# tensorflow/compression

Measured on NVIDIA H100. Metric: range-code throughput (bls2017 compress path, cfg2), higher is better.
Workload: dtype u32

## Files before the change

compression_b200/csrc/range_coder.cu:

```cuda
#include <algorithm>
#include <cstring>
#include <vector>

#include <cstring>
#include <mutex>
#include <vector>

#include "common.cuh"

namespace tfcb {
namespace {

constexpr unsigned kFull = 0xFFFFFFFFu;

struct HostRow {
  int32_t start;
  int32_t ncdf;
  int32_t prec;
};

__host__ __device__ inline int row_ncdf(int meta) { return meta & 0xFFFFFF; }
__host__ __device__ inline int row_prec(int meta) { return (meta >> 24) & 0x1F; }
__host__ __device__ inline bool row_ovf(int meta) { return meta < 0; }

// ... 78 lines not shown
    if (for_decoder) {
      hr4.resize(meta.size());
      for (size_t i = 0; i < hr.size(); ++i) {
        const int ap = hr[i].prec < 0 ? -hr[i].prec : hr[i].prec;
        const int n = hr[i].ncdf - 1;
        const int pstart = (int)hp.size();
        int median = n, irregular = 0;
        for (int e = 0; e <= n; ++e) {
          const uint32_t c = (uint32_t)lookup_host[hr[i].start + e];
          hp.push_back((c == (1u << ap)) ? make_uint2(0xFFFFFFFFu, 0u) : make_uint2(c << (32 - ap), 0xFFFFFFFFu));
          if (e >= 1 && c == 0u) irregular = 1;
          if (e >= 1 && e < n && c == (1u << ap)) irregular = 1;
          if (e >= 1 && median == n && c >= (1u << ap) / 2) median = e;
        }
        for (int e = n + 1; e <= 64; ++e) hp.push_back(make_uint2(0xFFFFFFFFu, 0u));
        int wfirst = median - 31;
        if (wfirst > n - 63) wfirst = n - 63;
        if (wfirst < 1) wfirst = 1;
        hr4[i] = make_int4(pstart, meta[i].y, wfirst, irregular);
      }
      zero_win = (int)hp.size();
      for (int e = 0; e < 64; ++e) hp.push_back(make_uint2(0u, 0u));
      n_pairs = (long long)hp.size();
      TFCB_TRY(dev_alloc((void**)&pairs, hp.size() * sizeof(uint2), s));
      TFCB_TRY(dev_alloc((void**)&rows4, hr4.size() * sizeof(int4), s));
      TFCB_CUDA_TRY(cudaMemcpyAsync(pairs, hp.data(), hp.size() * sizeof(uint2), cudaMemcpyHostToDevice, s));
      TFCB_CUDA_TRY(cudaMemcpyAsync(rows4, hr4.data(), hr4.size() * sizeof(int4), cudaMemcpyHostToDevice, s));
    }
    TFCB_CUDA_TRY(cudaStreamSynchronize(s));
    return TFCB_OK;
  }
  void release(cudaStream_t s) {
    dev_free(lookup, s);
    dev_free(rows, s);
    dev_free(pairs, s);
    dev_free(rows4, s);
    lookup = nullptr;
    rows = nullptr;
    pairs = nullptr;
    rows4 = nullptr;
  }
};

struct EncState {
  uint32_t base;
  uint32_t span;
  uint32_t cnt;
  uint32_t raw;
};

__host__ __device__ inline EncState enc_initial_state() {
  EncState s;
  s.base = 0;
  s.span = 0xFFFFFFFFu;
  s.cnt = 0;
  s.raw = 0xFFFFFFFFu;
  return s;
}


__device__ __forceinline__ uint4 enc_operands(uint32_t lower, uint32_t upper, uint32_t p) {
  const uint32_t sh = 16u - p;
  return make_uint4(lower << sh, 0u, upper << sh, 0u);
}

struct EncChain {
  uint32_t s;

  __device__ __forceinline__ uint2 step(uint2 ol, uint2 oh) {
    const unsigned long long ql = (unsigned long long)s * ol.x + (((unsigned long long)ol.y << 32) | ol.x);
    const unsigned long long qu = (unsigned long long)s * oh.x + (((unsigned long long)oh.y << 32) | oh.x);
    const uint32_t shift = (s < 65536u) ? 0u : 16u;
    const uint32_t L = __funnelshift_r((uint32_t)ql, (uint32_t)(ql >> 32), shift);
    const uint32_t U = __funnelshift_r((uint32_t)qu, (uint32_t)(qu >> 32), shift);
    asm("{\n\t.reg .u32 t;\n\tsub.u32 t, %1, %2;\n\tsub.u32 %0, t, 1;\n\t}" : "=r"(s) : "r"(U), "r"(L));
    return make_uint2(L, s);
  }
  __device__ __forceinline__ uint2 step(uint4 o) { return step(make_uint2(o.x, o.y), make_uint2(o.z, o.w)); }
};

__device__ __forceinline__ uint32_t shl_clamp(uint32_t x, uint32_t s) { return __funnelshift_lc(0u, x, s); }

struct EncDrain {
  uint32_t dbase;
  uint32_t cnt;
  uint32_t cb_cur;
  uint16_t* words;
  uint32_t* cbits;
  uint32_t cap;
  bool overflowed;
  int lane;

  __device__ __forceinline__ void begin(const EncState& st, uint16_t* w, uint32_t* cb, uint32_t cap_, int lane_) {
    dbase = st.base;
    cnt = st.cnt;
    words = w;
    cbits = cb;
    cap = cap_;
    overflowed = false;
    lane = lane_;
    cb_cur = (st.cnt == 0) ? 0u : cb[st.cnt >> 5];
  }

  template <int kPasses>
  __device__ __forceinline__ void drain(const uint2* ent, int n) {
    uint32_t Lk[kPasses], Ak[kPasses], Sk[kPasses], rmask[kPasses];
#pragma unroll
    for (int p = 0; p < kPasses; ++p) {
      const int k = p * 32 + lane;
      const bool act = k < n;
      const uint2 me = ent[act ? k : 0];
      const bool rr = act && me.y < 65536u;
      rmask[p] = __ballot_sync(kFull, rr);
      Lk[p] = act ? me.x : 0u;
      uint32_t S = rr ? 16u : 0u;
      uint32_t A = Lk[p] << S;
#pragma unroll
      for (int d = 1; d < 32; d <<= 1) {
        const uint32_t Ap = __shfl_up_sync(kFull, A, d);
        const uint32_t Sp = __shfl_up_sync(kFull, S, d);
        if (lane >= d) {
          A = shl_clamp(Ap, S) + A;
          S = min(Sp + S, 32u);
        }
      }
      Ak[p] = A;
      Sk[p] = S;
    }
#pragma unroll
    for (int p = 0; p < kPasses; ++p) {
      if (p * 32 >= n) break;
      uint32_t Ax = __shfl_up_sync(kFull, Ak[p], 1);
      uint32_t Sx = __shfl_up_sync(kFull, Sk[p], 1);
      if (lane == 0) {
        Ax = 0u;
        Sx = 0u;
      }
      const uint32_t before = shl_clamp(dbase, Sx) + Ax;
      const uint32_t nb = before + Lk[p];
      const bool carry = nb < before;
      const bool ren = (rmask[p] >> lane) & 1u;
      const uint32_t my_cnt = cnt + __popc(rmask[p] & ((1u << lane) - 1u));
      if (ren) {
        if (my_cnt < cap) words[my_cnt] = (uint16_t)(nb >> 16);
        else overflowed = true;
      }
      const uint32_t g0 = cnt >> 5;
      const uint32_t bit = 1u << (my_cnt & 31u);
      const uint32_t m0 = __reduce_or_sync(kFull, (carry && (my_cnt >> 5) == g0) ? bit : 0u);
      const uint32_t m1 = __reduce_or_sync(kFull, (carry && (my_cnt >> 5) != g0) ? bit : 0u);
      const uint32_t pass_end = cnt + __popc(rmask[p]);
      cb_cur |= m0;
      if ((pass_end >> 5) != g0) {
        if (lane == 0 && g0 < (cap >> 5)) cbits[g0] = cb_cur;
        cb_cur = m1;
      }
      cnt = pass_end;
      dbase = shl_clamp(dbase, __shfl_sync(kFull, Sk[p], 31)) + __shfl_sync(kFull, Ak[p], 31);
    }
  }

  __device__ __forceinline__ void end(DevError* err, long long stream) {
    if ((cnt >> 5) < (cap >> 5)) {
      if (lane == 0) cbits[cnt >> 5] = cb_cur;
    } else {
      overflowed = true;
    }
    if (__any_sync(kFull, overflowed)) report(err, kErrCapacity, stream, cnt, cnt, cap);
  }
};

enum : int { kModeIndex = 1, kModeF32 = 2, kModeDecoded = 4 };

struct EncParams {
  const int32_t* lookup;
  const int2* rows;
  int n_rows;
  int uniform_prec;
  const void* value;
  const int32_t* index;
  const float* qoff;
  const int32_t* coff;
  long long n;
  long long n_streams;
  int fresh;
  EncState* state;
  uint16_t* words;
  uint32_t* cbits;
  long long cap;
  DevError* err;
  const long long* sym_off;
  const long long* arena_off;
  float* decoded;
};

struct Extent {
  long long base, len;
};
__device__ __forceinline__ Extent stream_extent(const long long* off, long long s, long long stride) {
  if (off) return Extent{off[s], off[s + 1] - off[s]};
  return Extent{s * stride, stride};
}

struct Fetched {
  float y;
  int v;
  float loc_or_q;
  int coff;
  int row;
  int2 ri;
  bool valid;
};

struct Gathered {
  uint4 ops;
  uint32_t prec;
  uint32_t gamma;
  uint32_t sign;
};

template <int MODE>
__device__ __forceinline__ Fetched enc_fetch(const EncParams& P, long long end, long long at, uint32_t chan_row) {
  Fetched f;
  f.y = 0.f;
  f.v = 0;
  f.loc_or_q = 0.f;
  f.coff = 0;
  f.row = (int)chan_row;
  f.ri = make_int2(0, 0);
  f.valid = at < end;
  if (!f.valid) return f;
  if (MODE & kModeF32) {
    f.y = __ldg(reinterpret_cast<const float*>(P.value) + at);
  } else {
    f.v = __ldg(reinterpret_cast<const int32_t*>(P.value) + at);
  }
  if (MODE & kModeIndex) {
    f.row = __ldg(P.index + at);
    if ((MODE & kModeF32) && P.qoff) f.loc_or_q = __ldg(P.qoff + at);
  } else {
    f.ri = __ldg(P.rows + f.row);
    if (MODE & kModeF32) {
      if (P.qoff) f.loc_or_q = __ldg(P.qoff + f.row);
      f.coff = __ldg(P.coff + f.row);
    }
  }
  return f;
}

template <int MODE>
__device__ __forceinline__ Gathered enc_gather(const EncParams& P, long long s, long long at, Fetched f) {
  Gathered g;
  g.ops = make_uint4(0u, 0u, 0u, 0u);
  g.prec = 0;
  g.gamma = 0;
  g.sign = 0;
  if (!f.valid) return g;
  if (MODE & kModeIndex) {
    if (f.row < 0 || f.row >= P.n_rows) {
      report(P.err, kErrIndex, s, at - stream_extent(P.sym_off, s, P.n).base, f.row, P.n_rows);
      return g;
    }
    f.ri = __ldg(P.rows + f.row);
    if (MODE & kModeF32) f.coff = __ldg(P.coff + f.row);
  }
  int v = f.v;
  if (MODE & kModeF32) v = (int)rintf(f.y - f.loc_or_q) - f.coff;
  if (MODE & kModeDecoded) {
    float yv = (float)(v + f.coff);
    if (P.qoff) yv += f.loc_or_q;
    P.decoded[at] = yv;
  }
  const int ncdf = row_ncdf(f.ri.y);
  if (!row_ovf(f.ri.y)) {
    if (v < 0 || v >= ncdf - 1) {
      report(P.err, kErrValue, s, at - stream_extent(P.sym_off, s, P.n).base, v, ncdf - 1);
      return g;
    }
  } else {
    const int esc = ncdf - 2;
    if (v < 0) {
      g.gamma = (uint32_t)(-(long long)v);
      g.sign = 1;
      v = esc;
    } else if (v >= esc) {
      g.gamma = (uint32_t)(v - esc + 1);
      v = esc;
    }
  }
  const uint32_t lower = (uint32_t)__ldg(P.lookup + f.ri.x + v);
  const uint32_t upper = (uint32_t)__ldg(P.lookup + f.ri.x + v + 1);
  g.prec = (uint32_t)row_prec(f.ri.y);
  g.ops = enc_operands(lower, upper, g.prec);
  return g;
}

__device__ __forceinline__ void bar_sync(int id, int count) {
  asm volatile("bar.sync %0, %1;" ::"r"(id), "r"(count) : "memory");
}
__device__ __forceinline__ void bar_arrive(int id, int count) {
  asm volatile("bar.arrive %0, %1;" ::"r"(id), "r"(count) : "memory");
}

constexpr int kBlock = 256;

struct BlockInfo {
  uint32_t n;
  uint32_t last;
};

constexpr int kPrefetch = 4;
static_assert(kPrefetch == 2 || kPrefetch == 4 || kPrefetch == 8, "the chain loop unrolls by 8 records");

struct EncShared {
  uint4 ops[2][kBlock + kPrefetch];
  uint2 ent[2][kBlock];
  BlockInfo ops_info[2];
  BlockInfo ent_info[2];
};

enum : int { kBarOpsFull = 1, kBarOpsEmpty = 3, kBarEntFull = 5, kBarEntEmpty = 7 };

struct RecordWriter {
  EncShared* sh;
  long long blocks;
  int fill;

  __device__ __forceinline__ void begin(EncShared* sh_) {
    sh = sh_;
    blocks = 0;
    fill = 0;
  }
  __device__ __forceinline__ uint4* cur() { return sh->ops[blocks & 1]; }
  __device__ __forceinline__ void publish(bool last) {
    const int b = (int)(blocks & 1);
    if ((threadIdx.x & 31) == 0) {
      BlockInfo bi;
      bi.n = (uint32_t)fill;
      bi.last = last ? 1u : 0u;
      sh->ops_info[b] = bi;
    }
    bar_arrive(kBarOpsFull + b, 64);
    ++blocks;
    fill = 0;
    if (!last && blocks >= 2) bar_sync(kBarOpsEmpty + (int)(blocks & 1), 64);
  }
  template <typename F>
  __device__ __forceinline__ void append(uint4 first, int pre, int extra, int total, bool has, F rec) {
    int done = 0;
    while (done < total) {
      const int room = kBlock - fill;
      const int take = min(room, total - done);
      uint4* dst = cur() + fill - done;
      if (has) {
        if (pre >= done && pre < done + take) dst[pre] = first;
        for (int i = 0; i < extra; ++i) {
          const int at = pre + 1 + i;
          if (at >= done && at < done + take) dst[at] = rec(i);
        }
      }
      fill += take;
      done += take;
      if (fill == kBlock) publish(false);
    }
  }
};

__device__ __forceinline__ uint4 gamma_record(uint32_t g, uint32_t sign, int nb, int i) {
  uint32_t bit;
  if (i < nb - 1) bit = 0u;
  else if (i < 2 * nb - 1) bit = (g >> (2 * nb - 2 - i)) & 1u;
  else bit = sign;
  return enc_operands(bit, bit + 1u, 1u);
}

template <int MODE>
__global__ void __launch_bounds__(192) encode_kernel(const EncParams P) {
  __shared__ __align__(16) EncShared sh;
  const long long s = blockIdx.x;
  const int lane = threadIdx.x & 31;
  const int warp = threadIdx.x >> 5;
  if (warp != 0 && warp != 1 && warp != 5) return;

  if (warp == 1) {
    uint32_t row_a = 0, chan_step = 0;
    if (!(MODE & kModeIndex)) {
      row_a = (uint32_t)lane % (uint32_t)P.n_rows;
      chan_step = 32u % (uint32_t)P.n_rows;
    }
    auto advance_row = [&]() {
      if (!(MODE & kModeIndex)) {
        row_a += chan_step;
        if (row_a >= (uint32_t)P.n_rows) row_a -= (uint32_t)P.n_rows;
      }
    };
    const Extent x = stream_extent(P.sym_off, s, P.n);
    const long long end = x.base + x.len;
    Fetched f0 = enc_fetch<MODE>(P, end, x.base + lane, row_a);
    advance_row();
    Fetched f1 = enc_fetch<MODE>(P, end, x.base + 32 + lane, row_a);
    advance_row();
    Fetched f2 = enc_fetch<MODE>(P, end, x.base + 64 + lane, row_a);
    advance_row();
    RecordWriter w;
    w.begin(&sh);
    bool stop = false;
    for (long long j0 = x.base; j0 < end && !stop; j0 += 32) {
      const Fetched fcur = f0;
      f0 = f1;
      f1 = f2;
      f2 = enc_fetch<MODE>(P, end, j0 + 96 + lane, row_a);
      advance_row();
      const Gathered cur = enc_gather<MODE>(P, s, j0 + lane, fcur);
      const int count = (int)min(32ll, end - j0);
      const bool has = lane < count;
      const unsigned esc_mask = __ballot_sync(kFull, cur.gamma != 0);
      const unsigned bad_mask = __ballot_sync(kFull, cur.prec == 0 && has);
      if (bad_mask) {
        stop = true;
        break;
      }
      if (esc_mask == 0) {
        if (w.fill + count <= kBlock) {
          if (has) w.cur()[w.fill + lane] = cur.ops;
          w.fill += count;
          if (w.fill == kBlock) w.publish(false);
        } else {
          w.append(cur.ops, lane, 0, count, has, [&](int) { return cur.ops; });
        }
      } else {
        const int nb = cur.gamma ? 32 - __clz(cur.gamma) : 0;
        const int mine = has ? 1 + 2 * nb : 0;
        int incl = mine;
#pragma unroll
        for (int d = 1; d < 32; d <<= 1) {
          const int t = __shfl_up_sync(kFull, incl, d);
          if (lane >= d) incl += t;
        }
        const int total = __shfl_sync(kFull, incl, 31);
        w.append(cur.ops, incl - mine, 2 * nb, total, has,
                 [&](int i) { return gamma_record(cur.gamma, cur.sign, nb, i); });
      }
    }
    w.publish(true);
    return;
  }

  if (warp == 5) {
    EncDrain d;
    const Extent a = stream_extent(P.arena_off, s, P.cap);
    d.begin(P.fresh ? enc_initial_state() : P.state[s], P.words + a.base, P.cbits + (a.base >> 5), (uint32_t)a.len,
            lane);
    for (long long k = 0;; ++k) {
      const int b = (int)(k & 1);
      bar_sync(kBarEntFull + b, 64);
      const BlockInfo bi = sh.ent_info[b];
      d.drain<kBlock / 32>(sh.ent[b], (int)bi.n);
      if (bi.last) break;
      bar_arrive(kBarEntEmpty + b, 64);
    }
    d.end(P.err, s);
    if (lane == 0) {
      P.state[s].base = d.dbase;
      P.state[s].cnt = d.cnt;
    }
    return;
  }

  EncChain c;
  c.s = P.fresh ? enc_initial_state().raw : P.state[s].raw;
  for (long long k = 0;; ++k) {
    const int b = (int)(k & 1);
    bar_sync(kBarOpsFull + b, 64);
    const BlockInfo bi = sh.ops_info[b];
    if (k >= 2) bar_sync(kBarEntEmpty + b, 64);
    const uint2* q = reinterpret_cast<const uint2*>(sh.ops[b]);
    uint2* e = sh.ent[b];
    const int n = (int)bi.n;
    int kk = 0;
    uint2 lo[kPrefetch], hi[kPrefetch];
#pragma unroll
    for (int r = 0; r < kPrefetch; ++r) {
      lo[r] = q[2 * r];
      hi[r] = q[2 * r + 1];
    }
#pragma unroll 1
    for (; kk + 8 <= n; kk += 8) {
      const uint2* p = q + 2 * kk;
      uint2* const eo = e + kk;
#pragma unroll
      for (int j = 0; j < 8; j += 2) {
        const int r0 = j % kPrefetch, r1 = (j + 1) % kPrefetch;
        const uint2 a0 = lo[r0], b0 = hi[r0], a1 = lo[r1], b1 = hi[r1];
        lo[r0] = p[2 * (j + kPrefetch)];
        hi[r0] = p[2 * (j + kPrefetch) + 1];
        lo[r1] = p[2 * (j + 1 + kPrefetch)];
        hi[r1] = p[2 * (j + 1 + kPrefetch) + 1];
        eo[j] = c.step(a0, b0);
        eo[j + 1] = c.step(a1, b1);
      }
    }
    for (; kk < n; ++kk) e[kk] = c.step(sh.ops[b][kk]);
    if (lane == 0) sh.ent_info[b] = bi;
    bar_arrive(kBarEntFull + b, 64);
    if (bi.last) break;
    bar_arrive(kBarOpsEmpty + b, 64);
  }
  if (lane == 0) {
    P.state[s].span = (c.s < 65536u) ? ((c.s << 16) | 0xFFFFu) : c.s;
    P.state[s].raw = c.s;
  }
}

__global__ void enc_init_state_kernel(EncState* st, long long n) {
  const long long i = blockIdx.x * (long long)blockDim.x + threadIdx.x;
  if (i < n) st[i] = enc_initial_state();
}

__device__ __forceinline__ long long enc_final_length(const EncState& st, const uint16_t* words,
                                                      bool* straddle, uint32_t* tail, int* ntail) {
  const uint32_t top_end = st.base + st.span;
  *ntail = 0;
  *tail = 0;
  if (top_end < st.base) {
    *straddle = true;
    uint32_t d = st.cnt - 1u;
    while (d > 0 && words[d] == 0xFFFFu) --d;
    const uint32_t wd = ((uint32_t)words[d] + 1u) & 0xFFFFu;
    return 2ll * d + 1 + ((wd & 0xFFu) ? 1 : 0);
  }
  *straddle = false;
  if (st.base != 0) {
    const uint32_t r24 = ((st.base - 1u) >> 24) + 1u;
    if (r24 <= (top_end >> 24)) {
      *tail = r24 << 8;
      *ntail = 1;
    } else {
      const uint32_t r16 = ((st.base - 1u) >> 16) + 1u;
      *tail = r16;
      *ntail = (r16 & 0xFFu) ? 2 : 1;
    }
  }
  return 2ll * st.cnt + *ntail;
}

struct EncResult {
  long long total;
  DevError err;
};

struct EncArena {
  long long n_streams = 0;
  EncState* state = nullptr;
  uint16_t* words = nullptr;
  uint32_t* cbits = nullptr;
  long long cap = 0;
  DevError* err = nullptr;
  const long long* arena_off = nullptr;
};

__global__ void __launch_bounds__(1024) enc_offsets_kernel(const EncState* state, const uint16_t* words,
                                                           long long cap, const long long* arena_off,
                                                           long long n_streams, long long* offsets,
                                                           DevError* err, int reset_err, EncResult* res) {
  __shared__ long long warp_sums[32];
  __shared__ long long carry_s;
  const int tid = threadIdx.x, lane = tid & 31, wid = tid >> 5;
  if (tid == 0) carry_s = 0;
  __syncthreads();
  for (long long base = 0; base < n_streams; base += blockDim.x) {
    const long long i = base + tid;
    long long v = 0;
    if (i < n_streams) {
      bool straddle;
      uint32_t tail;
      int ntail;
      v = enc_final_length(state[i], words + (arena_off ? arena_off[i] : i * cap), &straddle, &tail, &ntail);
    }
    long long x = v;
#pragma unroll
    for (int d = 1; d < 32; d <<= 1) {
      const long long y = __shfl_up_sync(kFull, x, d);
      if (lane >= d) x += y;
    }
    if (lane == 31) warp_sums[wid] = x;
    __syncthreads();
    if (wid == 0) {
      long long w = (lane < (int)(blockDim.x >> 5)) ? warp_sums[lane] : 0;
#pragma unroll
      for (int d = 1; d < 32; d <<= 1) {
        const long long y = __shfl_up_sync(kFull, w, d);
        if (lane >= d) w += y;
      }
      warp_sums[lane] = w;
    }
    __syncthreads();
    const long long before = carry_s + (wid ? warp_sums[wid - 1] : 0) + (x - v);
    if (i < n_streams) offsets[i] = before;
    __syncthreads();
    if (tid == blockDim.x - 1) carry_s = before + v;
    __syncthreads();
  }
  if (tid == 0) {
    offsets[n_streams] = carry_s;
    res->total = carry_s;
    res->err = *err;
    if (reset_err) *err = DevError{};
  }
}

constexpr int kWriteWarps = 8;

__global__ void __launch_bounds__(32 * kWriteWarps) enc_write_kernel(const EncState* state, const uint16_t* words,
                                                                    const uint32_t* cbits, long long cap,
                                                                    const long long* arena_off, long long n_streams,
                                                                    const long long* offsets, uint8_t* out) {
  __shared__ uint32_t seg_out[kWriteWarps][2];
  const long long s = blockIdx.x;
  const int lane = threadIdx.x & 31, warp = threadIdx.x >> 5;
  if (s >= n_streams) return;
  const EncState st = state[s];
  const long long abase = arena_off ? arena_off[s] : s * cap;
  const uint16_t* w = words + abase;
  const uint32_t* cb = cbits + (abase >> 5);
  uint8_t* dst = out + offsets[s];
  bool straddle;
  uint32_t tail;
  int ntail;
  const long long len = enc_final_length(st, w, &straddle, &tail, &ntail);
  const long long body = straddle ? len : 2ll * st.cnt;

  const long long n_groups = ((long long)st.cnt + 31) >> 5;
  const long long per = (n_groups + kWriteWarps - 1) / kWriteWarps;
  const long long g_lo = min((long long)warp * per, n_groups), g_hi = min(g_lo + per, n_groups);
  const bool even = ((reinterpret_cast<uintptr_t>(dst)) & 1) == 0;
  constexpr int kBatch = 8;

  auto pass = [&](uint32_t& x0, uint32_t& x1, const bool write) {
    for (long long gt = g_hi; gt > g_lo; gt -= kBatch) {
      uint32_t word[kBatch], F[kBatch];
#pragma unroll
      for (int i = 0; i < kBatch; ++i) {
        const long long g = gt - 1 - i;
        const uint32_t idx = (uint32_t)(g << 5) + lane;
        word[i] = (g >= g_lo && idx < st.cnt) ? (uint32_t)w[idx] : 0u;
        F[i] = (g >= g_lo) ? cb[g] : 0u;
      }
#pragma unroll
      for (int i = 0; i < kBatch; ++i) {
        const long long g = gt - 1 - i;
        if (g < g_lo) break;
        const uint32_t idx = (uint32_t)(g << 5) + lane;
        const bool live = idx < st.cnt;
        uint32_t Fm = F[i];
        const uint32_t fill = st.cnt - (uint32_t)(g << 5);
        if (fill < 32u) Fm &= (1u << fill) - 1u;
        const uint32_t Pm = __ballot_sync(kFull, live ? (word[i] == 0xFFFFu) : true);
        const uint32_t G = __brev(Fm);
        const uint32_t A = G | __brev(Pm);
        const unsigned long long sum = (unsigned long long)A + G + x0;
        if (!write) x1 = (uint32_t)(((unsigned long long)A + G + x1) >> 32) & 1u;
        const uint32_t cin = (uint32_t)sum ^ A ^ G;
        const uint32_t my_c = (cin >> (31 - lane)) & 1u;
        x0 = (uint32_t)(sum >> 32) & 1u;
        if (write && live) {
          const uint32_t r = (word[i] + my_c) & 0xFFFFu;
          const long long b0 = 2ll * idx;
          if (even && b0 + 1 < body) {
            *reinterpret_cast<uint16_t*>(dst + b0) = (uint16_t)((r >> 8) | ((r & 0xFFu) << 8));
          } else {
            if (b0 < body) dst[b0] = (uint8_t)(r >> 8);
            if (b0 + 1 < body) dst[b0 + 1] = (uint8_t)r;
          }
        }
      }
    }
  };
  uint32_t o0 = 0u, o1 = 1u;
  pass(o0, o1, false);
  if (lane == 0) {
    seg_out[warp][0] = o0;
    seg_out[warp][1] = o1;
  }
  __syncthreads();
  uint32_t x = straddle ? 1u : ((cb[st.cnt >> 5] >> (st.cnt & 31u)) & 1u);
  for (int k = kWriteWarps - 1; k > warp; --k) x = seg_out[k][x];
  uint32_t unused = 0u;
  pass(x, unused, true);
  if (!straddle && threadIdx.x == 0) {
    if (ntail >= 1) dst[body] = (uint8_t)(tail >> 8);
    if (ntail == 2) dst[body + 1] = (uint8_t)tail;
  }
}

__global__ void enc_grow_kernel(const uint16_t* src, const uint32_t* src_cb, long long src_cap,
                                uint16_t* dst, uint32_t* dst_cb, long long dst_cap,
                                const EncState* state) {
  const long long s = blockIdx.x;
  const uint32_t used = (state[s].cnt + 31u) & ~31u;
  for (uint32_t i = threadIdx.x; i < used; i += blockDim.x) dst[s * dst_cap + i] = src[s * src_cap + i];
  for (uint32_t i = threadIdx.x; i <= (state[s].cnt >> 5); i += blockDim.x)
    dst_cb[s * (dst_cap >> 5) + i] = src_cb[s * (src_cap >> 5) + i];
}

struct DecState {
  uint32_t base, span, value;
  uint32_t pos;
};

struct DecParams {
  const int32_t* lookup;
  const int2* rows;
  const uint2* pairs;
  const int4* rows4;
  int n_rows;
  long long lookup_len;
  long long n_pairs;
  int zero_win;
  const uint8_t* bytes;
  const long long* offsets;
  const int32_t* index;
  void* out;
  const float* qoff;
  const int32_t* coff;
  long long n;
  long long n_streams;
  DecState* state;
  DevError* err;
  const long long* sym_off;
};

struct ByteWindow {
  const uint8_t* p;
  long long len;
  uint32_t lane_word;
  uint32_t next;
};

__device__ __forceinline__ uint32_t bw_fetch(const ByteWindow& w, long long word_idx) {
  const long long b = 2 * word_idx;
  uint32_t hi = 0, lo = 0;
  if (b < w.len) hi = w.p[b];
  if (b + 1 < w.len) lo = w.p[b + 1];
  return (hi << 8) | lo;
}

__device__ __forceinline__ void bw_seek(ByteWindow& w, uint32_t pos, int lane) {
  w.lane_word = bw_fetch(w, (long long)(pos & ~31u) + lane);
  w.next = __shfl_sync(kFull, w.lane_word, pos & 31u);
}

struct DecChain {
  uint32_t base, span, value, pos;
};

__device__ __forceinline__ void dec_update(DecChain& c, ByteWindow& w, uint32_t a, uint32_t b, int lane) {
  c.base += a;
  c.span = b - a - 1u;
  if (c.span < 65536u) {
    c.base <<= 16;
    c.span = (c.span << 16) | 0xFFFFu;
    c.value = (c.value << 16) | w.next;
    c.pos += 1;
    if ((c.pos & 31u) == 0) {
      bw_seek(w, c.pos, lane);
    } else {
      w.next = __shfl_sync(kFull, w.lane_word, c.pos & 31u);
    }
  }
}

__device__ __forceinline__ int dec_symbol(DecChain& c, ByteWindow& w, const int32_t* cdf, int ncdf,
                                          uint32_t p, int lane) {
  const uint32_t v = c.value - c.base;
  int lo_i = 1;
  int n = ncdf - 1;
  int i;
  for (;;) {
    const int stride = (n + 31) >> 5;
    int off = (lane + 1) * stride - 1;
    if (off > n - 1) off = n - 1;
    const uint32_t cv = (uint32_t)cdf[lo_i + off];
    const bool pred = v < scale_cum(c.span, cv, p);
    const bool full = (cv == (1u << p)) && (c.span == 0xFFFFFFFFu);
    const unsigned m = __ballot_sync(kFull, pred || full);
    const int f = m ? (__ffs(m) - 1) : 31;
    if (stride == 1) {
      i = lo_i + min(f, n - 1);
      break;
    }
    const int skip = min(f * stride, n - 1);
    lo_i += skip;
    n = min(stride, n - skip);
  }
  const uint32_t ca = (uint32_t)cdf[i - 1];
  const uint32_t cb = (uint32_t)cdf[i];
  dec_update(c, w, scale_cum(c.span, ca, p), scale_cum(c.span, cb, p), lane);
  return i - 1;
}


constexpr int kDecGroup = 128;
constexpr int kRing = 2048;
constexpr int kRingAhead = 1536;

struct DecDesc {
  int win;
  uint32_t thr;
  int seg;
// ... 1516 lines not shown
```

Baseline: 13610.

## Triple-buffer the encoder warp pipeline and enlarge record blocks

Extends the producer/chain/drain warp-specialized encoder pipeline from double to triple buffering, with buffer indices rotating through next_buf. The named barrier ids are generalized so each buffer gets its own full and empty barriers. It also raises the block size from 256 to 384 records. The aim is to absorb rate jitter between stages so fewer warps stall on barrier waits. In exchange it uses more shared memory per CTA (ops are uint4 records), which may lower occupancy.

Measured after the change: 14780 (median of 6 runs). 1.09x the previous value.

```diff
diff --git a/compression_b200/csrc/range_coder.cu b/compression_b200/csrc/range_coder.cu
--- a/compression_b200/csrc/range_coder.cu
+++ b/compression_b200/csrc/range_coder.cu
@@ -404,7 +404,9 @@
   asm volatile("bar.arrive %0, %1;" ::"r"(id), "r"(count) : "memory");
 }
 
-constexpr int kBlock = 256;
+constexpr int kBlock = 384;
+constexpr int kBufs = 3;
+static_assert(4 * kBufs < 16, "four named barriers per buffer, id 0 is __syncthreads");
 
 struct BlockInfo {
   uint32_t n;
@@ -415,27 +417,36 @@
 static_assert(kPrefetch == 2 || kPrefetch == 4 || kPrefetch == 8, "the chain loop unrolls by 8 records");
 
 struct EncShared {
-  uint4 ops[2][kBlock + kPrefetch];
-  uint2 ent[2][kBlock];
-  BlockInfo ops_info[2];
-  BlockInfo ent_info[2];
-};
-
-enum : int { kBarOpsFull = 1, kBarOpsEmpty = 3, kBarEntFull = 5, kBarEntEmpty = 7 };
+  uint4 ops[kBufs][kBlock + kPrefetch];
+  uint2 ent[kBufs][kBlock];
+  BlockInfo ops_info[kBufs];
+  BlockInfo ent_info[kBufs];
+};
+
+enum : int {
+  kBarOpsFull = 1,
+  kBarOpsEmpty = 1 + kBufs,
+  kBarEntFull = 1 + 2 * kBufs,
+  kBarEntEmpty = 1 + 3 * kBufs
+};
+
+__device__ __forceinline__ int next_buf(int b) { return b + 1 == kBufs ? 0 : b + 1; }
 
 struct RecordWriter {
   EncShared* sh;
   long long blocks;
+  int buf;
   int fill;
 
   __device__ __forceinline__ void begin(EncShared* sh_) {
     sh = sh_;
     blocks = 0;
+    buf = 0;
     fill = 0;
   }
-  __device__ __forceinline__ uint4* cur() { return sh->ops[blocks & 1]; }
+  __device__ __forceinline__ uint4* cur() { return sh->ops[buf]; }
   __device__ __forceinline__ void publish(bool last) {
-    const int b = (int)(blocks & 1);
+    const int b = buf;
     if ((threadIdx.x & 31) == 0) {
       BlockInfo bi;
       bi.n = (uint32_t)fill;
@@ -444,8 +455,9 @@
     }
     bar_arrive(kBarOpsFull + b, 64);
     ++blocks;
+    buf = next_buf(buf);
     fill = 0;
-    if (!last && blocks >= 2) bar_sync(kBarOpsEmpty + (int)(blocks & 1), 64);
+    if (!last && blocks >= kBufs) bar_sync(kBarOpsEmpty + buf, 64);
   }
   template <typename F>
   __device__ __forceinline__ void append(uint4 first, int pre, int extra, int total, bool has, F rec) {
@@ -553,8 +565,7 @@
     const Extent a = stream_extent(P.arena_off, s, P.cap);
     d.begin(P.fresh ? enc_initial_state() : P.state[s], P.words + a.base, P.cbits + (a.base >> 5), (uint32_t)a.len,
             lane);
-    for (long long k = 0;; ++k) {
-      const int b = (int)(k & 1);
+    for (int b = 0;; b = next_buf(b)) {
       bar_sync(kBarEntFull + b, 64);
       const BlockInfo bi = sh.ent_info[b];
       d.drain<kBlock / 32>(sh.ent[b], (int)bi.n);
@@ -571,11 +582,11 @@
 
   EncChain c;
   c.s = P.fresh ? enc_initial_state().raw : P.state[s].raw;
+  int b = 0;
   for (long long k = 0;; ++k) {
-    const int b = (int)(k & 1);
     bar_sync(kBarOpsFull + b, 64);
     const BlockInfo bi = sh.ops_info[b];
-    if (k >= 2) bar_sync(kBarEntEmpty + b, 64);
+    if (k >= kBufs) bar_sync(kBarEntEmpty + b, 64);
     const uint2* q = reinterpret_cast<const uint2*>(sh.ops[b]);
     uint2* e = sh.ent[b];
     const int n = (int)bi.n;
@@ -607,6 +618,7 @@
     bar_arrive(kBarEntFull + b, 64);
     if (bi.last) break;
     bar_arrive(kBarOpsEmpty + b, 64);
+    b = next_buf(b);
   }
   if (lane == 0) {
     P.state[s].span = (c.s < 65536u) ? ((c.s << 16) | 0xFFFFu) : c.s;
```
